# ChrisHird/ZLIB

Hardware: AMD Instinct MI355X
Metric: GiB/s raw input compressed (deflate level 6) (higher is better)
Workload: dtype u8

## Files before the change

### zlib_amd/csrc/zgpu_lz_parse.h

```cpp
#pragma once
#include "zgpu_common.h"

namespace zgpu {

#ifndef ZGPU_P2WIN
#define ZGPU_P2WIN 8192
#endif
constexpr uint32_t kP2Win = ZGPU_P2WIN, kP2Blk = kP2Win / 64;
constexpr uint32_t kP2Words = kChunkMax / 32, kP2Batch = 8, kP2Pair = 4, kP2Over = 8;
constexpr uint32_t kNone = 0xffffffffu;

struct ParseCtx {
    const uint2 *rec;
    uint32_t n, base, good, lazy, strategy;
    int slide_at;
    __device__ bool slid(uint32_t p) const { return (int)p >= slide_at; }
    __device__ uint32_t take(uint32_t p, uint32_t prev_len, uint2 r, uint32_t &dist) const
    {
        const uint32_t pick = (prev_len >= good && strategy != kRle) ? r.y : r.x;
        const uint32_t d = (pick >> 9) & 32767u;
        const bool nil = ((r.y >> 24) & 1u) && slid(p);
        const uint32_t len = nil ? 0u : (pick & 511u);
        const bool weak = len <= 5 && (strategy == kFiltered || (len == kMinMatch && d > kTooFar));
        const bool ok = prev_len < lazy && len > prev_len && !weak;
// ... 7 lines not shown
        uint32_t q = r + 1;
        for (;;) {
            uint32_t D2 = 0;
            const uint32_t L2 = take(q, L, rn, D2);
            if (L2 <= L) break;
            L = L2; D = D2; q++;
            rn = rec[q];
        }
        m = q - 1; len = L; dist = D;
    }
};

__device__ inline uint32_t wave_rol1(uint32_t v) { return (uint32_t)__builtin_amdgcn_update_dpp(0, (int)v, 0x134, 0xf, 0xf, false); }

__device__ inline uint32_t next_bit(const uint32_t *bits, uint32_t x, uint32_t nwords)
{
    uint32_t w = x >> 5;
    if (w >= nwords) return kNone;
    uint32_t v = bits[w] & (~0u << (x & 31u));
    while (v == 0) { if (++w >= nwords) return kNone; v = bits[w]; }
    return (w << 5) + (uint32_t)__builtin_ctz(v);
}

#if defined(ZGPU_P2_TIME) && !defined(ZGPU_PARSE_HEADER_ONLY)
__device__ unsigned long long p2_time[8];
extern "C" __attribute__((visibility("default"))) void zgpu_debug_p2_time(unsigned long long *out, int reset)
{
    unsigned long long z[8] = {};
    hipMemcpyFromSymbol(out, HIP_SYMBOL(p2_time), sizeof z);
    if (reset) hipMemcpyToSymbol(HIP_SYMBOL(p2_time), z, sizeof z);
}
#define P2_T(i) do { if (tid == 0) { const unsigned long long t_ = wall_clock64(); t_acc[i] += t_ - t_prev; t_prev = t_; } } while (0)
#define P2_T0() unsigned long long t_prev = wall_clock64(), t_acc[8] = {0, 0, 0, 0, 0, 0, 0, 0}
#define P2_TEND() do { if (tid == 0) for (int i_ = 0; i_ < 8; i_++) atomicAdd(&p2_time[i_], t_acc[i_]); } while (0)
#else
#define P2_T(i) do { } while (0)
#define P2_T0() do { } while (0)
#define P2_TEND() do { } while (0)
#endif

template <bool FUSED> __device__ inline uint32_t p2_ld(const uint32_t *p) { return FUSED ? __hip_atomic_load(p, __ATOMIC_RELAXED, __HIP_MEMORY_SCOPE_AGENT) : *p; }
constexpr uint32_t kP2OffJ = 0, kP2OffHAS = kP2Win * 2, kP2OffMARK = kP2OffHAS + kP2Words * 4, kP2OffCOV = kP2OffMARK + kP2Words * 4, kP2OffMAT = kP2OffCOV + kP2Words * 4,
                   kP2OffWbase = kP2OffMAT + kP2Words * 4, kP2OffVIS = kP2OffWbase + (kP2Words + 4) * 4, kP2OffEXITS = kP2OffVIS + kP2Win / 32 * 4, kP2OffWtot = kP2OffEXITS + 256,
                   kP2OffEntry = kP2OffWtot + 64, kP2LdsBytes = kP2OffEntry + 16;
constexpr uint32_t kP2Wins = kChunkMax / kP2Win, kP2OffEND = kP2LdsBytes, kP2LogLdsBytes = kP2OffEND + kP2Win * 2;
static_assert(kChunkMax % kP2Win == 0 && kP2Win - 1 + 255 + 258 <= 0xffffu, "whole windows; a game's end fits END");

}
```

### zlib_amd/csrc/zgpu_lz_parse_body.inc

```
{
    constexpr uint32_t kP2Own = kP2Win / kP2Threads;
    static_assert(kP2Own % kP2Batch == 0 && kP2Threads >= kP2Win / 32 && kP2Threads / 64 <= 16, "workgroup size");
    const uint32_t tid = threadIdx.x, lane = tid & 63, wave = tid >> 6;
    uint64_t lo; uint32_t n;
    chunk_span(g, c, lo, n);
    ParseCtx cx;
    cx.rec = LITE ? nullptr : recs + (size_t)c * kChunkMax;
    const uint32_t *gmv = LITE ? gmv_all + (size_t)c * kChunkMax : nullptr, *gsv = LITE ? gsv_all + (size_t)c * kP2Words : nullptr;
    cx.n = n; cx.base = chunk_base(g, c); cx.good = cfg.good; cx.lazy = cfg.lazy; cx.strategy = cfg.strategy;
    {
        const int room = (int)(2 * kWSize - cx.base), b0 = (int)n < room ? (int)n : room;
        const int a = b0 - (int)kMinLookahead + 1, b = (int)(kWSize + kMaxDist) - (int)cx.base;
        cx.slide_at = a > b ? a : b;
    }
    uint32_t *tok = tokens + (size_t)c * kChunkMax;
    const uint8_t *src = g.in + lo;
    const uint32_t nwords = (n + 31) >> 5;
    uint32_t t_h1 = n, t_e = 0;
    if (TILE) {
        uint64_t wb_; uint32_t nl_, h0_, ne_;
        tile_span(g, tg, c, wb_, nl_, h0_, t_h1, ne_);
        t_e = h0_ + tg.entry[g.chunk0 + c];
    }

    static_assert(!LOG || (LITE && !TILE), "the logs are what a chunk's walkers leave");
    P2_T0();
    for (uint32_t i = tid; i < kP2Words; i += kP2Threads) { MARK[i] = 0; COV[i] = 0; MAT[i] = 0; if (LOG) HAS[i] = 0; else if (LITE) HAS[i] = p2_ld<FUSED>(gsv + i); }
    const uint32_t *lpos2 = reinterpret_cast<const uint32_t *>(lpos);
    if (LOG) {
        constexpr uint32_t kRounds = kP2Win / 2 / kP2Threads;
        __syncthreads();
        for (uint32_t w = 0; w < kP2Wins; w++) {
            const uint32_t cw = (uint32_t)__builtin_amdgcn_readfirstlane((int)lcnt[w]);
            uint32_t pv[kRounds];
#pragma unroll
            for (uint32_t r = 0; r < kRounds; r++) { pv[r] = 0; if (r * kP2Threads * 2 < cw) pv[r] = p2_ld<FUSED>(lpos2 + w * (kP2Win / 2) + r * kP2Threads + tid); }
#pragma unroll
            for (uint32_t r = 0; r < kRounds; r++) {
                const uint32_t e = (r * kP2Threads + tid) * 2, p0 = pv[r] & 0xffffu, p1 = pv[r] >> 16;
                if (e < cw) atomicOr(&HAS[p0 >> 5], 1u << (p0 & 31u));
                if (e + 1 < cw) atomicOr(&HAS[p1 >> 5], 1u << (p1 & 31u));
            }
        }
    }
    if (!LITE) for (uint32_t p0 = 0; p0 < kChunkMax; p0 += kP2Threads * kP2Batch) {
        uint2 rv[kP2Batch];
#pragma unroll
        for (uint32_t u = 0; u < kP2Batch; u++) { const uint32_t p = p0 + u * kP2Threads + tid; rv[u] = p < n ? cx.rec[p] : make_uint2(0, 0); }
#pragma unroll
        for (uint32_t u = 0; u < kP2Batch; u++) {
            const uint32_t pw = p0 + u * kP2Threads, p = pw + tid;
            uint32_t d;
            const bool h = p < n && cx.take(p, kMinMatch - 1, rv[u], d) >= kMinMatch;
            const unsigned long long b = __builtin_amdgcn_ballot_w64(h);
            if (lane == 0) { HAS[(pw >> 5) + 2 * wave] = (uint32_t)b; HAS[(pw >> 5) + 2 * wave + 1] = (uint32_t)(b >> 32); }
        }
    }
    __syncthreads();
    if (tid == 0) {
        uint32_t x0 = (!TILE || t_e < t_h1) ? next_bit(HAS, t_e, nwords) : kNone;
        if (TILE && x0 != kNone && x0 >= t_h1) x0 = kNone;
        sh_entry = x0;
        if (TILE) sh_exit = t_e;
    }
    __syncthreads();
    P2_T(0);

    const uint32_t *TOK = COV;
    auto index_of = [&](uint32_t p) { return wbase[p >> 5] + (uint32_t)__builtin_popcount(TOK[p >> 5] & ~(~0u << (p & 31u))); };
    uint32_t tokbase = 0;
    uint32_t def_m = kNone, def_tok = 0;

    const uint32_t w_first = TILE ? t_e / kP2Win * kP2Win : 0u, w_lim = TILE ? (t_h1 + kTileSlack < n ? t_h1 + kTileSlack : n) : n;
    for (uint32_t w0 = w_first; w0 < w_lim; w0 += kP2Win) {
        const uint32_t wend = w0 + kP2Win;
        const uint32_t entry = sh_entry;
        uint32_t gm[kP2Own];
        uint32_t gp[kP2Own];
        uint32_t onp = 0;
#pragma unroll
        for (uint32_t i = 0; i < kP2Own; i++) { gm[i] = 0; gp[i] = 0; }
        auto pos_of = [&](uint32_t i) { return LOG ? gp[i] : w0 + i * kP2Threads + tid; };
        if (entry != kNone && entry < wend) {
            if (LOG) {
                const uint32_t cw = (uint32_t)__builtin_amdgcn_readfirstlane((int)lcnt[w0 / kP2Win]);
                const uint32_t *lp2 = lpos2 + w0 / 2, *lr = lrec + w0;
                uint32_t gv[kP2Own], gq[kP2Own];
#pragma unroll
                for (uint32_t i = 0; i < kP2Own; i++) {
                    gv[i] = 0; gq[i] = 0;
                    if (i * kP2Threads < cw) { const uint32_t e = i * kP2Threads + tid; gq[i] = p2_ld<FUSED>(lp2 + (e >> 1)); gv[i] = p2_ld<FUSED>(lr + e); }
                }
#pragma unroll
                for (uint32_t i = 0; i < kP2Own; i++) {
                    const bool v = i * kP2Threads + tid < cw;
                    const uint32_t p = (gq[i] >> ((tid & 1u) << 4)) & 0xffffu;
                    gm[i] = v ? gv[i] : 0u; gp[i] = v ? p : 0u;
                    if (v) {
                        const uint32_t end = p + (gv[i] >> 24) + ((gv[i] >> 15) & 511u), t = next_bit(HAS, end, nwords);
                        J[p - w0] = (uint16_t)(t < wend ? t - w0 : 0xffffu);
                        END[p - w0] = (uint16_t)(end - w0);
                    }
                }
            } else if (LITE) {
                uint32_t gv[kP2Own];
#pragma unroll
                for (uint32_t i = 0; i < kP2Own; i++) {
                    const uint32_t p = w0 + i * kP2Threads + tid;
#if defined(ZGPU_P2_EXP) && ZGPU_P2_EXP == 1
                    gv[i] = 0x00018001u;
#else
                    gv[i] = p < n ? p2_ld<FUSED>(gmv + p) : 0;
#endif
                }
#pragma unroll
                for (uint32_t i = 0; i < kP2Own; i++) {
                    const uint32_t p = w0 + i * kP2Threads + tid;
                    if (!(p < n && ((HAS[p >> 5] >> (p & 31u)) & 1u))) gv[i] = 0;
                }
#pragma unroll
                for (uint32_t i = 0; i < kP2Own; i++) {
                    const uint32_t xw = i * kP2Threads + tid, p = w0 + xw;
// ... 28 lines not shown
                        const uint32_t tx = wave_rol1(qx), ty = wave_rol1(qy);
                        ox = wave_rol1(ox); oy = wave_rol1(oy);
                        qx = lane == 63 ? ox : tx; qy = lane == 63 ? oy : ty;
                        uint2 rn;
                        rn.x = qx; rn.y = qy;
                        const bool far = live && sl >= 64 + kP2Over;
                        if (__builtin_amdgcn_ballot_w64(far)) { if (far) rn = cx.rec[p + j]; }
                        uint32_t D2 = D;
                        const uint32_t L2 = cx.take(p + j, L, rn, D2);
                        live = live && L2 > L;
                        L = live ? L2 : L; D = live ? D2 : D; j += live ? 1u : 0u;
                    }
                    uint32_t succ = 0xffffu;
                    if (hs) {
                        const uint32_t m = p + j - 1;
                        gm[ib + u] = ((m - p) << 24) | (L << 15) | D;
                        const uint32_t t = next_bit(HAS, m + L, nwords);
                        if (t < wend) succ = t - w0;
                    }
                    J[x] = (uint16_t)succ;
                }
            }
            }
            __syncthreads();
            P2_T(1);
            if (wave == 0) {
                const uint32_t bs = w0 + lane * kP2Blk, be = bs + kP2Blk;
                uint32_t v8[kP2Blk / 32];
#pragma unroll
                for (uint32_t j = 0; j < kP2Blk / 32; j++) v8[j] = 0;
                uint32_t x = next_bit(HAS, bs, nwords);
                if (x != kNone && x >= wend) x = kNone;
                while (x != kNone && x < be) {
                    const uint32_t wi = (x - bs) >> 5, bit = 1u << (x & 31u);
#pragma unroll
                    for (uint32_t j = 0; j < kP2Blk / 32; j++) v8[j] |= wi == j ? bit : 0u;
                    const uint32_t a2 = J[x - w0];
                    x = a2 == 0xffffu ? kNone : w0 + a2;
                }
#pragma unroll
                for (uint32_t j = 0; j < kP2Blk / 32; j++) VIS[lane * (kP2Blk / 32) + j] = v8[j];
                EXITS[lane] = x;
                __builtin_amdgcn_fence(__ATOMIC_SEQ_CST, "wavefront");
                __builtin_amdgcn_wave_barrier();
                uint32_t last = entry;
                bool ok;
// ... 108 lines not shown
            uint32_t tw = 0;
            if (tid < kP2Win / 32 && wd < nwords) {
                tw = ~COV[wd];
                if (wd == nwords - 1 && (n & 31u)) tw &= ~0u >> (32u - (n & 31u));
                if (TILE) {
                    const uint32_t xl = wend > t_h1 ? (sh_exit > t_h1 ? sh_exit : t_h1) : wend, p0 = wd << 5;
                    tw &= p0 + 32 <= t_e ? 0u : p0 >= t_e ? ~0u : ~0u << (t_e & 31u);
                    tw &= p0 >= xl ? 0u : p0 + 32 <= xl ? ~0u : ~0u >> (32u - (xl & 31u));
                }
            }
            const uint32_t cnt = (uint32_t)__builtin_popcount(tw);
            uint32_t x = cnt;
#pragma unroll
            for (int d = 1; d < 64; d <<= 1) { const uint32_t y = __shfl_up(x, d); if ((int)lane >= d) x += y; }
            if (lane == 63) wave_tot[wave] = x;
            __syncthreads();
            uint32_t b = tokbase + x - cnt, tot = 0;
            for (uint32_t w = 0; w < kP2Win / 32 / 64; w++) { const uint32_t t = wave_tot[w]; tot += t; if (w < wave) b += t; }
            if (tid < kP2Win / 32) { wbase[wd] = b; COV[wd] = tw; }
            tokbase += tot;
            __syncthreads();
        }
        P2_T(4);
        if (def_m != kNone) { tok[index_of(def_m)] = def_tok; def_m = kNone; }
#pragma unroll
        for (uint32_t ib = 0; ib < kP2Own; ib += kP2Batch) {
            uint32_t lit[kP2Batch];
            bool li[kP2Batch];
#pragma unroll
            for (uint32_t u = 0; u < kP2Batch; u++) {
                const uint32_t p = w0 + (ib + u) * kP2Threads + tid, bit = 1u << (p & 31u);
                li[u] = p < n && (TOK[p >> 5] & bit) && !(MAT[p >> 5] & bit);
                lit[u] = 0;
                if (p < n) lit[u] = src[p];
            }
#pragma unroll
            for (uint32_t u = 0; u < kP2Batch; u++) {
                const uint32_t p = w0 + (ib + u) * kP2Threads + tid;
                if (li[u]) tok[index_of(p)] = tok_lit(lit[u]);
                const uint32_t gv = (!LOG && ((onp >> (ib + u)) & 1u)) ? gm[ib + u] : 0u;
                if (gv) {
                    const uint32_t m = p + (gv >> 24), t = tok_match(gv & 32767u, ((gv >> 15) & 511u) - kMinMatch);
                    if (m < wend) tok[index_of(m)] = t; else { def_m = m; def_tok = t; }
                }
            }
        }
        if (LOG) {
#pragma unroll
            for (uint32_t i = 0; i < kP2Own; i++) {
                const uint32_t gv = ((onp >> i) & 1u) ? gm[i] : 0u;
                if (gv) {
                    const uint32_t m = gp[i] + (gv >> 24), t = tok_match(gv & 32767u, ((gv >> 15) & 511u) - kMinMatch);
                    if (m < wend) tok[index_of(m)] = t; else { def_m = m; def_tok = t; }
                }
            }
        }
        P2_T(5);
    }
    const uint32_t ntok = tokbase, nw_done = ((n + kP2Win - 1) / kP2Win) * (kP2Win / 32);
    __syncthreads();

    if (TILE) { if (tid == 0) { meta[c].ntok = ntok; meta[c].in_bytes = (sh_exit > t_h1 ? sh_exit : t_h1) - t_e; } }
    else if (tid == 0) {
        uint32_t nostore = 0, nblk = 0, block_start = 0;
        for (uint32_t b = 0;; b++) {
            const uint32_t e = (b + 1) * kBlockTokens - 1;
            if (e >= ntok) break;
            uint32_t lo_w = 0, hi_w = nw_done;
            while (hi_w - lo_w > 1) { const uint32_t mid = (lo_w + hi_w) >> 1; if (wbase[mid] <= e) lo_w = mid; else hi_w = mid; }
            uint32_t v = TOK[lo_w];
            for (uint32_t s2 = e - wbase[lo_w]; s2; s2--) v &= v - 1;
            const uint32_t pe = (lo_w << 5) + (uint32_t)__builtin_ctz(v);
            const bool is_mat = (MAT[pe >> 5] >> (pe & 31u)) & 1u;
            if (!is_mat && pe == n - 1) { nostore |= kFullFinalBlock; break; }
            uint32_t ns = pe + 1;
            if (is_mat) { ns = next_bit(TOK, pe + 1, nwords); if (ns == kNone) ns = n; }
            if (cx.slid(pe + 1) && block_start + cx.base < kWSize) nostore |= 1u << nblk;
            nblk++; block_start = ns;
// ... 8 lines not shown
```

### zlib_amd/csrc/zgpu_lz_sorted.hip

```cpp
#include "zgpu_common.h"
#include "zgpu_engine.h"
#include "zgpu_deflate_batch_plan.h"
#define ZGPU_PARSE_HEADER_ONLY
#include "zgpu_lz_parse.h"
#include <cstdlib>
#include "../../include/zamd_gpu.h"

#include <atomic>
static std::atomic<int> g_inject_sort_fault{0};
extern "C" __attribute__((visibility("default"))) void zgpu_debug_inject_sort_fault(void) { g_inject_sort_fault.store(1); }

namespace zgpu {

__device__ inline uint32_t lds_off(const void *p) { return (uint32_t)(uintptr_t)(const __attribute__((address_space(3))) void *)p; }
__device__ inline void lds_st32(uint32_t a, uint32_t v) { asm volatile("ds_write_b32 %0, %1" ::"v"(a), "v"(v) : "memory"); }
__device__ inline void lds_st16(uint32_t a, uint32_t v) { asm volatile("ds_write_b16 %0, %1" ::"v"(a), "v"(v) : "memory"); }
__device__ inline void lds_max32(uint32_t a, uint32_t v) { asm volatile("ds_max_u32 %0, %1" ::"v"(a), "v"(v) : "memory"); }
__device__ inline uint32_t lds_ld32(uint32_t a) { uint32_t v; asm volatile("ds_read_b32 %0, %1\n\ts_waitcnt lgkmcnt(0)" : "=v"(v) : "v"(a) : "memory"); return v; }
__device__ inline uint32_t lds_ld16(uint32_t a) { uint32_t v; asm volatile("ds_read_u16 %0, %1\n\ts_waitcnt lgkmcnt(0)" : "=v"(v) : "v"(a) : "memory"); return v; }

__device__ inline void lds_st8(uint32_t a, uint32_t v) { asm volatile("ds_write_b8 %0, %1" ::"v"(a), "v"(v) : "memory"); }
__device__ inline uint32_t lds_ld8(uint32_t a) { uint32_t v; asm volatile("ds_read_u8 %0, %1\n\ts_waitcnt lgkmcnt(0)" : "=v"(v) : "v"(a) : "memory"); return v; }

constexpr uint32_t kSuperS = 1024;
// ... 639 lines not shown
            uint32_t full = 0, snap = 0, flags = 0;
            if (key_seen) {
                const uint32_t kb = 4095u - ((key_seen >> 31) ? (key_seen >> 16) & 0xfffu : key_seen & 0xfffu);
                full = best | ((p - (uint32_t)sp[-1 - (int)kb]) << 9);
            }
            if (snapkey) {
                const uint32_t ks = 4095u - ((snapkey >> 31) ? (snapkey >> 16) & 0xfffu : snapkey & 0xfffu);
                const uint32_t sl = (snapkey >> 31) ? snapkey & 0x1ffu : snapkey >> 16;
                snap = sl | ((p - (uint32_t)sp[-1 - (int)ks]) << 9);
            }
            if (p + base == kWSize + kMaxDist && avail != 0 && (uint32_t)sp[-1] + base == kWSize) flags = 1;
            rec[p] = make_uint2(full | ((uint32_t)d8[p] << 24), snap | (flags << 24));
        }
        blk = blk_nx;
    }
}

#ifndef ZGPU_WTRIG
#define ZGPU_WTRIG 48
#endif
#ifndef ZGPU_WBLK
#define ZGPU_WBLK 64
#endif
#ifndef ZGPU_WNEU_SHIFT
#define ZGPU_WNEU_SHIFT 0
#endif
#ifndef ZGPU_WFOLD_AT
#define ZGPU_WFOLD_AT 64
#endif
constexpr uint32_t kWFoldAt = ZGPU_WFOLD_AT;
constexpr uint32_t kWThreads = 512, kWWaves = kWThreads / 64, kWBlk = ZGPU_WBLK, kWTrig = ZGPU_WTRIG, kWNeuShift = ZGPU_WNEU_SHIFT;
constexpr uint32_t kWNeuBytes = (kChunkMax >> kWNeuShift) / 8;
constexpr uint32_t kWOffLcnt = kM3DataLds + 16 + kWNeuBytes + kWWaves * kM3WaveLds;
constexpr uint32_t kWLds = kWOffLcnt + kP2Wins * 4;
static_assert(2 * kWLds <= 160 * 1024, "two walker workgroups per CU");
enum : uint32_t { W_NEED = 0, W_LIMBO = 1, W_READY = 2, W_SEARCH = 3, W_DONE = 4 };
#ifdef ZGPU_WALK_STATS
__device__ unsigned long long walk_stats[8];
extern "C" __attribute__((visibility("default"))) void zgpu_debug_walk_stats(unsigned long long *out, int reset)
{
    unsigned long long z[8] = {};
    hipMemcpyFromSymbol(out, HIP_SYMBOL(walk_stats), sizeof z);
    if (reset) hipMemcpyToSymbol(HIP_SYMBOL(walk_stats), z, sizeof z);
}
#define W_STAT(i, v) do { const unsigned long long v_ = (unsigned long long)(v); if (lane == 0) atomicAdd(&walk_stats[i], v_); } while (0)
__device__ unsigned long long walk_log_stats[2];
extern "C" __attribute__((visibility("default"))) void zgpu_debug_walk_log_stats(unsigned long long *out, int reset)
{
    unsigned long long z[2] = {};
    hipMemcpyFromSymbol(out, HIP_SYMBOL(walk_log_stats), sizeof z);
    if (reset) hipMemcpyToSymbol(HIP_SYMBOL(walk_log_stats), z, sizeof z);
}
#else
#define W_STAT(i, v) do { } while (0)
#endif
#ifdef ZGPU_WALK_TIME
__device__ unsigned long long walk_time[8];
extern "C" __attribute__((visibility("default"))) void zgpu_debug_walk_time(unsigned long long *out, int reset)
{
    unsigned long long z[8] = {};
    hipMemcpyFromSymbol(out, HIP_SYMBOL(walk_time), sizeof z);
    if (reset) hipMemcpyToSymbol(HIP_SYMBOL(walk_time), z, sizeof z);
}
#define W_T0() unsigned long long wt_prev = __builtin_readcyclecounter(), wt_fold = 0, wt_lds = 0, wt_take = 0, wt_acc[8] = {0, 0, 0, 0, 0, 0, 0, 0}
#define W_T(i) do { const unsigned long long t_ = __builtin_readcyclecounter(); wt_acc[i] += t_ - wt_prev - ((i) == 1 ? wt_fold + wt_lds + wt_take : 0); \
                    if ((i) == 1) { wt_acc[2] += wt_fold; wt_acc[3] += wt_lds; wt_acc[7] += wt_take; } wt_fold = wt_lds = wt_take = 0; wt_prev = t_; } while (0)
#define W_TF(stmt) do { const unsigned long long f0_ = __builtin_readcyclecounter(); stmt; wt_fold += __builtin_readcyclecounter() - f0_; } while (0)
#define W_TL(stmt) do { const unsigned long long f0_ = __builtin_readcyclecounter(); stmt; wt_lds += __builtin_readcyclecounter() - f0_; } while (0)
#define W_TK(stmt) do { const unsigned long long f0_ = __builtin_readcyclecounter(); asm volatile("s_waitcnt vmcnt(0)" ::: "memory"); stmt; wt_take += __builtin_readcyclecounter() - f0_; } while (0)
#define W_TEND() do { if (lane == 0) for (int i_ = 0; i_ < 8; i_++) atomicAdd(&walk_time[i_], wt_acc[i_]); } while (0)
#else
#define W_T0() do { } while (0)
#define W_T(i) do { } while (0)
#define W_TF(stmt) stmt
#define W_TL(stmt) stmt
#define W_TK(stmt) stmt
#define W_TEND() do { } while (0)
#endif
__device__ inline uint32_t add_w1(uint32_t b, uint32_t w) { uint32_t r; asm("v_add_u32_sdwa %0, %1, %2 dst_sel:DWORD dst_unused:UNUSED_PAD src0_sel:DWORD src1_sel:WORD_1" : "=v"(r) : "v"(b), "v"(w)); return r; }
__device__ inline uint32_t add_w0(uint32_t b, uint32_t w) { uint32_t r; asm("v_add_u32_sdwa %0, %1, %2 dst_sel:DWORD dst_unused:UNUSED_PAD src0_sel:DWORD src1_sel:WORD_0" : "=v"(r) : "v"(b), "v"(w)); return r; }
__device__ inline uint32_t or_w1(uint32_t b, uint32_t w) { uint32_t r; asm("v_or_b32_sdwa %0, %1, %2 dst_sel:DWORD dst_unused:UNUSED_PAD src0_sel:DWORD src1_sel:WORD_1" : "=v"(r) : "v"(b), "v"(w)); return r; }
__device__ inline uint32_t and_or(uint32_t w, uint32_t m, uint32_t b) { uint32_t r; asm("v_and_or_b32 %0, %1, %2, %3" : "=v"(r) : "v"(w), "s"(m), "v"(b)); return r; }
__device__ inline uint32_t sel_mask(unsigned long long m, uint32_t if_set, uint32_t if_clear) { uint32_t r; asm("v_cndmask_b32_e64 %0, %1, %2, %3" : "=v"(r) : "v"(if_clear), "v"(if_set), "s"(m)); return r; }

template <uint32_t T>
__device__ inline void tile_exits(uint8_t *pl, const uint32_t *gm, const uint32_t *gs, uint32_t h0, uint32_t h1, uint32_t nent, uint16_t *exits, uint32_t tid)
{
    constexpr uint32_t kWords = kChunkMax / 32;
    static_assert(kWords % T == 0 && T % 64 == 0 && T <= 1024, "workgroup size");
    uint32_t *HAS = reinterpret_cast<uint32_t *>(pl);
    uint16_t *wcnt = reinterpret_cast<uint16_t *>(pl + kWords * 4);
    uint32_t *wtot = reinterpret_cast<uint32_t *>(pl + kWords * 6);
    uint16_t *N = reinterpret_cast<uint16_t *>(pl + kWords * 6 + 64);
    constexpr uint32_t kCapNodes = (kM3DataLds - (kWords * 6 + 64)) / 2;
    static_assert(kCapNodes < 0x8000u && kCapNodes > kTileH1 / 3, "a path's game starts are three positions apart at least; different paths' need not be");
    const uint32_t lane = tid & 63, wave = tid >> 6;
    constexpr uint32_t per = kWords / T;
    uint32_t sum = 0, cnt[per];
#pragma unroll
    for (uint32_t i = 0; i < per; i++) {
// ... 78 lines not shown
    uint32_t *ctrl = lds + kM3DataLds / 4;
    uint32_t *NEU = ctrl + 4;
    uint32_t *lcnt = lds + kWOffLcnt / 4;
    const uint32_t c = blockIdx.x, tid = threadIdx.x, lane = tid & 63, wave = tid >> 6;
    const uint32_t ring = (uint32_t)__builtin_amdgcn_readfirstlane(lds_off(lds) + kM3DataLds + 16 + kWNeuBytes + wave * kM3WaveLds), slot = ring + kRing * 4;
    uint64_t lo; uint32_t n;
    chunk_span(g, c, lo, n);
    const uint8_t *src = g.in + lo;
    const uint16_t *S = S_all + (size_t)c * kSStride + kSPad;
    const uint32_t *ir = ir_all + (size_t)c * kChunkMax;
    uint32_t *gm = gm_all + (size_t)c * kChunkMax, *gs = gs_all + (size_t)c * (kChunkMax / 32);
    uint32_t *lrec = gm; uint16_t *lpos = reinterpret_cast<uint16_t *>(gs_all) + (size_t)c * kChunkMax;
    uint32_t th0 = 0, th1 = n, tnent = 0, tnent_all = 0, nil_local = ~0u;
    uint32_t base = chunk_base(g, c);
    if (TILE) {
        uint64_t wb; uint32_t nl;
        tile_span(g, tg, c, wb, nl, th0, th1, tnent);
        tnent_all = tnent;
        if (tnent > th1 - th0) tnent = th1 - th0;
        base = (tg.abs0_nil && tg.abs0 + wb == 0) ? 0u : 1u;
        if (tg.nil_pos >= wb && tg.nil_pos - wb < kChunkMax) nil_local = (uint32_t)(tg.nil_pos - wb);
    }
    const uint32_t npos = n >= 3 ? n - 2 : 0;
    stage_chunk<kWThreads>(src, n, d32, tid);
    for (uint32_t i = tid; i < kChunkMax / 32; i += kWThreads) { if (i < kWNeuBytes / 4) NEU[i] = 0; if (!FUSE) gs[i] = 0; }
    if (tid < 8) d32[(kChunkMax + 64) / 4 + tid] = 0xffffffffu;
    if (tid == 0) ctrl[0] = 0;
    if (FUSE && tid < kP2Wins) lcnt[tid] = 0;
    __syncthreads();
    int slide_at;
    {
        const int room = (int)(2 * kWSize - base), b0 = (int)n < room ? (int)n : room;
        const int a = b0 - (int)kMinLookahead + 1, b = (int)(kWSize + kMaxDist) - (int)base;
        slide_at = a > b ? a : b;
    }
    const uint32_t chainF = cfg.chain, chainQ = cfg.chain >> 2, dbase = lds_off(d32), nblk = TILE ? tnent + (th1 - th0 - tnent + kWBlk - 1) / kWBlk : (n + kWBlk - 1) / kWBlk;
    const uint32_t wlim = TILE ? th1 : n;
    const bool vexact = (chainF & 7u) != 0 || (chainQ & 7u) != 0 || cfg.strategy == kRle;
    uint32_t lanebits = lane << 16;
    const uint32_t dummy = ring + (kRing - 1) * 4;
    uint32_t st = W_NEED, x = 0, handL = kMinMatch - 1, handM = 0, handD = 0, gstart = 0;
    uint32_t irx = 0, irn = 0, irE = 0, irl = 0;
    bool haveE = false;
    uint32_t rem = 0, best = kMinMatch - 1, key_seen = 0, sentinel = 0, boff = dbase + 1;
    uint32_t sw0 = 0, sw1 = 0;
    int gi = -(int)kSPad;
    uint32_t firstb = 0;
    uint4 G0 = make_uint4(0, 0, 0, 0), G1 = G0, G2 = G0, G3 = G0, F0 = G0, F1 = G0, F2 = G0, F3 = G0;
    uint32_t left = 0;
    bool cont = false;
    unsigned long long amask = 0, jmask = 0;
    uint32_t tail = 0;

    auto fold = [&]() {
        const uint32_t cnt = tail < 64 ? tail : 64;
        W_STAT(5, 1); W_STAT(6, cnt);
        tail = (uint32_t)__builtin_amdgcn_readfirstlane(tail - cnt);
        const uint32_t e = lds_ld32(ring + ((tail + lane) << 2));
        const uint32_t q = e & 0xffffu, o = (e >> 16) & 63u, qa = dbase + q;
// ... 9 lines not shown
        if (lane < cnt) {
            const uint32_t look = n - po, cap = look < kMaxMatch ? look : kMaxMatch, nice = cfg.nice < look ? cfg.nice : look;
            const bool reach = po - q <= kMaxDist - ((e >> 22) & 1u ? 0u : 1u) && q + base >= 1u;
            uint32_t l = 0;
            while ((xa | xb) == 0 && l + 8 < cap) {
                l += 8;
                lds_cmp8(qa + l, dbase + po + l, xa, xb);
            }
            uint32_t len = xa ? l + ((uint32_t)__builtin_ctz(xa) >> 3) : xb ? l + 4 + ((uint32_t)__builtin_ctz(xb) >> 3) : l + 8;
            len = len < cap ? len : cap;
            if (len >= kMinMatch && reach) lds_max32(slot + o * 4, (len >= nice && len > (e >> 23)) ? (0x80000000u | (q << 9) | len) : ((len << 16) | q));
        }
        const uint32_t key = lds_ld32(slot + lane * 4);
        if (key != key_seen) {
            key_seen = key;
            best = (key >> 31) ? key & 0x1ffu : key >> 16;
            boff = dbase + best - 1;
        }
        amask &= ~mask_lt_i32((int)key, 0);
    };
    auto gload = [&](int gi) -> uint4 { gi = gi < -(int)kSPad ? -(int)kSPad : gi; return reinterpret_cast<const U128u *>(S + gi)->v; };

    W_T0();
    W_T(3);
    for (;;) {
        while (tail) fold();
        W_T(4);
        if (cont && (key_seen >> 31)) cont = false;
        const bool fin = st == W_SEARCH && !(((amask | jmask) >> lane) & 1ull) && !cont;
        W_STAT(2, 1); W_STAT(3, __popcll(__builtin_amdgcn_ballot_w64(fin || st == W_LIMBO || st == W_NEED)));
        if (st == W_LIMBO) { irx = irl; st = W_READY; }
        uint32_t y = 0, irY = 0, rec = 0;
        bool toN = false, haveIr = false, emit = false;
        if (fin) {
            uint32_t len = kMinMatch - 1, dist = 0;
            if (key_seen != sentinel) {
                const bool nz = key_seen >> 31;
                len = nz ? key_seen & 0x1ffu : key_seen >> 16;
                dist = x - (nz ? (key_seen >> 9) & 0xffffu : key_seen & 0xffffu);
            }
            if (len <= 5 && (cfg.strategy == kFiltered || (len == kMinMatch && dist > kTooFar))) len = kMinMatch - 1;
            if (len > handL) {
                if (handL < kMinMatch) gstart = x;
                handL = len; handD = dist; handM = x;
                if (len < cfg.lazy && x + 1 < npos) { x = x + 1; irx = irn; st = W_READY; }
                else emit = true;
                haveE = false;
            } else if (handL >= kMinMatch) emit = true;
            else { y = x + 1; irY = irn; toN = haveIr = true; }
            if (emit) {
                rec = ((handM - gstart) << 24) | (handL << 15) | handD;
                if (!FUSE) {
                    gm[gstart] = rec;
// ... 22 lines not shown
            const uint32_t at = lw * kP2Win + lslot;
            lrec[at] = rec; lpos[at] = (uint16_t)gstart;
        }
        if (toN) {
            st = W_NEED;
            if (y < wlim && (!meet || !(yold & ybit))) {
                x = y;
                if (haveIr) { irx = irY; st = W_READY; }
                else { irl = y < npos ? ir[y] : 0; st = W_LIMBO; W_STAT(7, 1); }
            }
        }
        W_T(5);
        {
            const unsigned long long nm = __builtin_amdgcn_ballot_w64(st == W_NEED);
            if (nm) {
                const int first = __builtin_ctzll(nm);
                uint32_t b0 = 0;
                if ((int)lane == first) b0 = atomicAdd(&ctrl[0], (uint32_t)__popcll(nm));
                b0 = (uint32_t)__builtin_amdgcn_readlane((int)b0, first);
                if (st == W_NEED) {
                    const uint32_t b = b0 + __builtin_amdgcn_mbcnt_hi((uint32_t)(nm >> 32), __builtin_amdgcn_mbcnt_lo((uint32_t)nm, 0));
                    if (b >= nblk) st = W_DONE;
                    else {
                        const uint32_t y2 = TILE ? (b < tnent ? th0 + b : th0 + tnent + (b - tnent) * kWBlk) : b * kWBlk, bit = 1u << ((y2 >> kWNeuShift) & 31u);
                        if (!(atomicOr(&NEU[(y2 >> kWNeuShift) >> 5], bit) & bit)) { x = y2; handL = kMinMatch - 1; irl = y2 < npos ? ir[y2] : 0; st = W_LIMBO; }
                    }
                }
            }
        }
        W_T(6);
        bool fresh = false;
        if (st == W_READY) {
            const uint32_t seed = handL, idx = irx & 0xffffu, rank = irx >> 16, budget = seed >= cfg.good ? (chainQ ? chainQ : 0xffffu) : chainF;
            uint32_t avail = (x < npos && seed < cfg.lazy) ? (rank < budget ? rank : budget) : 0;
            irn = x + 1 < npos ? ir[x + 1] : 0;
            if (seed >= kMinMatch) { const uint32_t E = handM + handL; irE = E < npos ? ir[E] : 0; haveE = true; }
            if (TILE) {
                if (x == nil_local && avail != 0 && x - (uint32_t)S[idx - 1] == kMaxDist) avail = 0;
                if (cfg.strategy == kHuffmanOnly) avail = 0;
                if (cfg.strategy == kRle && avail != 0) avail = x - (uint32_t)S[idx - 1] == 1 ? 1u : 0u;
            }
            else if (x + base == kWSize + kMaxDist && avail != 0 && (int)x >= slide_at && (uint32_t)S[idx - 1] + base == kWSize) avail = 0;
            best = seed; sentinel = (seed << 16) | 0xffffu; key_seen = sentinel; boff = dbase + best - 1;
            lds_st32(slot + lane * 4, sentinel);
            sw0 = tw0; sw1 = tw1;
            lanebits = (lane << 16) | (seed << 23);
            rem = avail; firstb = 1u << 22;
            gi = (int)idx - 8;
            st = W_SEARCH;
            fresh = avail != 0;
            W_STAT(4, 1);
        }
        if (cont) { cont = false; fresh = true; }
        jmask = __builtin_amdgcn_ballot_w64(fresh);
        if (fresh) {
            F0 = gload(gi);
            if (rem > 8) F1 = gload(gi - 8);
            if (rem > 16) F2 = gload(gi - 16);
            if (rem > 24) F3 = gload(gi - 24);
            gi -= 32;
        }
        W_T(0);
        if (__builtin_amdgcn_ballot_w64(st != W_DONE) == 0) { W_TEND(); break; }
        const unsigned long long smask = __builtin_amdgcn_ballot_w64(st == W_SEARCH);
        const uint32_t idle = (uint32_t)__popcll(__builtin_amdgcn_ballot_w64(st == W_LIMBO || st == W_NEED));

        for (bool first = true;; first = false) {
            const unsigned long long amask0 = amask;
            if (amask) {
                W_STAT(0, 1);
                uint32_t bb[8], a[8], boff_e, as;
                boff_e = boff; as = boff + x;
                if (!vexact) {
                    const uint32_t boff_i = dbase + kChunkMax + 8u;
                    G0.x = sel_mask(amask0, G0.x, 0u); G0.y = sel_mask(amask0, G0.y, 0u); G0.z = sel_mask(amask0, G0.z, 0u); G0.w = sel_mask(amask0, G0.w, 0u);
                    boff_e = sel_mask(amask0, boff, boff_i); as = sel_mask(amask0, as, boff_i + 64u);
                }
                a[0] = add_w1(boff_e, G0.w); a[1] = add_w0(boff_e, G0.w); a[2] = add_w1(boff_e, G0.z); a[3] = add_w0(boff_e, G0.z);
                a[4] = add_w1(boff_e, G0.y); a[5] = add_w0(boff_e, G0.y); a[6] = add_w1(boff_e, G0.x); a[7] = add_w0(boff_e, G0.x);
                uint32_t hi[8], s0, s1;
                W_TL(
                    asm volatile("ds_read_u8 %0, %18\n\tds_read_u8 %8, %18 offset:1\n\tds_read_u8 %1, %19\n\tds_read_u8 %9, %19 offset:1\n\t"
                                 "ds_read_u8 %2, %20\n\tds_read_u8 %10, %20 offset:1\n\tds_read_u8 %3, %21\n\tds_read_u8 %11, %21 offset:1\n\t"
                                 "ds_read_u8 %4, %22\n\tds_read_u8 %12, %22 offset:1\n\tds_read_u8 %5, %23\n\tds_read_u8 %13, %23 offset:1\n\t"
                                 "ds_read_u8 %6, %24\n\tds_read_u8 %14, %24 offset:1\n\tds_read_u8 %7, %25\n\tds_read_u8 %15, %25 offset:1\n\t"
                                 "ds_read_u8 %16, %26\n\tds_read_u8 %17, %26 offset:1\n\t"
// ... 54 lines not shown
                    while (tail >= kWFoldAt) W_TF(fold());
                }
                amask &= mask_gt_u32(rem, 8u);
                firstb = sel_mask(amask0, 0u, firstb);
            }
            G0 = G1; G1 = G2; G2 = G3;
            left = left ? left - 1 : 0;
            if (first && jmask) {
                W_TK(if ((jmask >> lane) & 1ull) { G0 = F0; G1 = F1; G2 = F2; G3 = F3; left = 4; });
            }
            rem = sel_mask(amask0, rem > 8 ? rem - 8 : 0, rem);
            {
                const unsigned long long cm = amask & mask_eq_u32(left, 0u);
                cont = cont || ((cm >> lane) & 1ull);
                amask &= ~cm;
            }
            amask |= jmask; jmask = 0;
            if (amask == 0 || (uint32_t)__popcll(smask & ~amask) + idle >= kWTrig) break;
        }
        W_T(1);
    }
    if (TILE) {
        __syncthreads();
        tile_exits<kWThreads>(reinterpret_cast<uint8_t *>(lds), gm, gs, th0, th1, tnent_all, tg.exits + (size_t)c * kTileExitStride, tid);
    }
    if (FUSE) {
        __syncthreads();
#ifdef ZGPU_WALK_STATS
        if (tid < kP2Wins) { atomicAdd(&walk_log_stats[0], (unsigned long long)lcnt[tid]); atomicMax(&walk_log_stats[1], (unsigned long long)lcnt[tid]); }
#endif
        constexpr uint32_t kP2Threads = kWThreads;
        constexpr bool LITE = true, FUSED = true, TILE = false, LOG = true;
        const uint2 *recs = nullptr;
        const uint32_t *gmv_all = nullptr, *gsv_all = nullptr;
        uint8_t *pl = reinterpret_cast<uint8_t *>(lds);
        uint16_t *const J = reinterpret_cast<uint16_t *>(pl + kP2OffJ);
        uint32_t *const HAS = reinterpret_cast<uint32_t *>(pl + kP2OffHAS), *const MARK = reinterpret_cast<uint32_t *>(pl + kP2OffMARK), *const COV = reinterpret_cast<uint32_t *>(pl + kP2OffCOV),
                 *const MAT = reinterpret_cast<uint32_t *>(pl + kP2OffMAT), *const wbase = reinterpret_cast<uint32_t *>(pl + kP2OffWbase), *const VIS = reinterpret_cast<uint32_t *>(pl + kP2OffVIS),
                 *const EXITS = reinterpret_cast<uint32_t *>(pl + kP2OffEXITS), *const wave_tot = reinterpret_cast<uint32_t *>(pl + kP2OffWtot);
        uint32_t &sh_entry = *reinterpret_cast<uint32_t *>(pl + kP2OffEntry), &sh_exit = *reinterpret_cast<uint32_t *>(pl + kP2OffEntry + 4);
        uint16_t *const END = reinterpret_cast<uint16_t *>(pl + kP2OffEND);
#include "zgpu_lz_parse_body.inc"
    }
}

struct __attribute__((packed, aligned(1))) U128b { uint4 v; };
enum : uint32_t { F_IR = 0, F_GROUP, F_CAND, F_EXT, F_DONE };

__device__ inline uint32_t first_diff16(uint4 a, uint4 b)
{
// ... 254 lines not shown
```

Baseline: 29.40.

## Prefetch next window's logs, batch token stores, and taper walker block sizes

The parse body now prefetches the next window's log entries and the current window's literal bytes while the current window is processed, so global loads overlap with compute. Token stores are batched, with indices computed first and then stored, and gp is packed two positions per register to cut VGPR use. The walker also splits the end of each chunk into smaller 32- and 16-byte blocks to shorten tail latency. Extra timing and stat instrumentation is added. These changes trade more live registers, from prefetched arrays and unrolled log loads, for less memory stall and less tail imbalance.

```diff
diff --git a/zlib_amd/csrc/zgpu_lz_parse.h b/zlib_amd/csrc/zgpu_lz_parse.h
--- a/zlib_amd/csrc/zgpu_lz_parse.h
+++ b/zlib_amd/csrc/zgpu_lz_parse.h
@@ -53,7 +53,9 @@
     return (w << 5) + (uint32_t)__builtin_ctz(v);
 }
 
-#if defined(ZGPU_P2_TIME) && !defined(ZGPU_PARSE_HEADER_ONLY)
+#ifdef ZGPU_P2_TIME
+#ifndef ZGPU_PARSE_HEADER_ONLY
+#define P2_TIME_ARR p2_time
 __device__ unsigned long long p2_time[8];
 extern "C" __attribute__((visibility("default"))) void zgpu_debug_p2_time(unsigned long long *out, int reset)
 {
@@ -61,9 +63,10 @@
     hipMemcpyFromSymbol(out, HIP_SYMBOL(p2_time), sizeof z);
     if (reset) hipMemcpyToSymbol(HIP_SYMBOL(p2_time), z, sizeof z);
 }
+#endif
 #define P2_T(i) do { if (tid == 0) { const unsigned long long t_ = wall_clock64(); t_acc[i] += t_ - t_prev; t_prev = t_; } } while (0)
 #define P2_T0() unsigned long long t_prev = wall_clock64(), t_acc[8] = {0, 0, 0, 0, 0, 0, 0, 0}
-#define P2_TEND() do { if (tid == 0) for (int i_ = 0; i_ < 8; i_++) atomicAdd(&p2_time[i_], t_acc[i_]); } while (0)
+#define P2_TEND() do { if (tid == 0) for (int i_ = 0; i_ < 7; i_++) atomicAdd(&P2_TIME_ARR[i_], t_acc[i_]); } while (0)
 #else
 #define P2_T(i) do { } while (0)
 #define P2_T0() do { } while (0)
diff --git a/zlib_amd/csrc/zgpu_lz_parse_body.inc b/zlib_amd/csrc/zgpu_lz_parse_body.inc
--- a/zlib_amd/csrc/zgpu_lz_parse_body.inc
+++ b/zlib_amd/csrc/zgpu_lz_parse_body.inc
@@ -27,19 +27,34 @@
     P2_T0();
     for (uint32_t i = tid; i < kP2Words; i += kP2Threads) { MARK[i] = 0; COV[i] = 0; MAT[i] = 0; if (LOG) HAS[i] = 0; else if (LITE) HAS[i] = p2_ld<FUSED>(gsv + i); }
     const uint32_t *lpos2 = reinterpret_cast<const uint32_t *>(lpos);
+    uint32_t nq[kP2Own], nv[kP2Own];
+    auto log_fetch = [&](uint32_t w0n, uint32_t tid) {
+        const uint32_t cw = (uint32_t)__builtin_amdgcn_readfirstlane((int)lcnt[w0n / kP2Win]);
+        const uint32_t *lp2 = lpos2 + w0n / 2, *lr = lrec + w0n;
+#pragma unroll
+        for (uint32_t i = 0; i < kP2Own; i++) {
+            nq[i] = 0; nv[i] = 0;
+            if (i * kP2Threads < cw) { const uint32_t e = i * kP2Threads + tid; nq[i] = p2_ld<FUSED>(lp2 + (e >> 1)); nv[i] = p2_ld<FUSED>(lr + e); }
+        }
+    };
     if (LOG) {
         constexpr uint32_t kRounds = kP2Win / 2 / kP2Threads;
         __syncthreads();
-        for (uint32_t w = 0; w < kP2Wins; w++) {
-            const uint32_t cw = (uint32_t)__builtin_amdgcn_readfirstlane((int)lcnt[w]);
-            uint32_t pv[kRounds];
-#pragma unroll
-            for (uint32_t r = 0; r < kRounds; r++) { pv[r] = 0; if (r * kP2Threads * 2 < cw) pv[r] = p2_ld<FUSED>(lpos2 + w * (kP2Win / 2) + r * kP2Threads + tid); }
+        log_fetch(0, tid);
+        uint32_t pv[kP2Wins][kRounds], cw[kP2Wins];
+#pragma unroll
+        for (uint32_t a = 0; a < kP2Wins; a++) {
+            cw[a] = (uint32_t)__builtin_amdgcn_readfirstlane((int)lcnt[a]);
+#pragma unroll
+            for (uint32_t r = 0; r < kRounds; r++) { pv[a][r] = 0; if (r * kP2Threads * 2 < cw[a]) pv[a][r] = p2_ld<FUSED>(lpos2 + a * (kP2Win / 2) + r * kP2Threads + tid); }
+        }
+#pragma unroll
+        for (uint32_t a = 0; a < kP2Wins; a++) {
 #pragma unroll
             for (uint32_t r = 0; r < kRounds; r++) {
-                const uint32_t e = (r * kP2Threads + tid) * 2, p0 = pv[r] & 0xffffu, p1 = pv[r] >> 16;
-                if (e < cw) atomicOr(&HAS[p0 >> 5], 1u << (p0 & 31u));
-                if (e + 1 < cw) atomicOr(&HAS[p1 >> 5], 1u << (p1 & 31u));
+                const uint32_t e = (r * kP2Threads + tid) * 2, p0 = pv[a][r] & 0xffffu, p1 = pv[a][r] >> 16;
+                if (e < cw[a]) atomicOr(&HAS[p0 >> 5], 1u << (p0 & 31u));
+                if (e + 1 < cw[a]) atomicOr(&HAS[p1 >> 5], 1u << (p1 & 31u));
             }
         }
     }
@@ -72,32 +87,36 @@
     uint32_t def_m = kNone, def_tok = 0;
 
     const uint32_t w_first = TILE ? t_e / kP2Win * kP2Win : 0u, w_lim = TILE ? (t_h1 + kTileSlack < n ? t_h1 + kTileSlack : n) : n;
+    const uint32_t tid_all = tid;
     for (uint32_t w0 = w_first; w0 < w_lim; w0 += kP2Win) {
         const uint32_t wend = w0 + kP2Win;
+        uint32_t tid = tid_all;
+        if (LOG) asm volatile("" : "+v"(tid));
         const uint32_t entry = sh_entry;
         uint32_t gm[kP2Own];
-        uint32_t gp[kP2Own];
+        uint32_t gp[kP2Own / 2];
         uint32_t onp = 0;
 #pragma unroll
-        for (uint32_t i = 0; i < kP2Own; i++) { gm[i] = 0; gp[i] = 0; }
-        auto pos_of = [&](uint32_t i) { return LOG ? gp[i] : w0 + i * kP2Threads + tid; };
-        if (entry != kNone && entry < wend) {
+        for (uint32_t i = 0; i < kP2Own; i++) { gm[i] = 0; gp[i >> 1] = 0; }
+        auto pos_of = [&](uint32_t i) { return LOG ? (gp[i >> 1] >> ((i & 1u) << 4)) & 0xffffu : w0 + i * kP2Threads + tid; };
+        uint32_t litw[kP2Own];
+        auto win_fetch = [&]() {
+#pragma unroll
+            for (uint32_t i = 0; i < kP2Own; i++) { const uint32_t p = w0 + i * kP2Threads + tid; litw[i] = 0; if (p < n) litw[i] = src[p]; }
+            if (wend < n) log_fetch(wend, tid);
+        };
+        const bool has_path = entry != kNone && entry < wend;
+        if (has_path) {
             if (LOG) {
                 const uint32_t cw = (uint32_t)__builtin_amdgcn_readfirstlane((int)lcnt[w0 / kP2Win]);
-                const uint32_t *lp2 = lpos2 + w0 / 2, *lr = lrec + w0;
-                uint32_t gv[kP2Own], gq[kP2Own];
-#pragma unroll
-                for (uint32_t i = 0; i < kP2Own; i++) {
-                    gv[i] = 0; gq[i] = 0;
-                    if (i * kP2Threads < cw) { const uint32_t e = i * kP2Threads + tid; gq[i] = p2_ld<FUSED>(lp2 + (e >> 1)); gv[i] = p2_ld<FUSED>(lr + e); }
-                }
 #pragma unroll
                 for (uint32_t i = 0; i < kP2Own; i++) {
                     const bool v = i * kP2Threads + tid < cw;
-                    const uint32_t p = (gq[i] >> ((tid & 1u) << 4)) & 0xffffu;
-                    gm[i] = v ? gv[i] : 0u; gp[i] = v ? p : 0u;
+                    const uint32_t p = (nq[i] >> ((tid & 1u) << 4)) & 0xffffu;
+                    const uint32_t gvi = nv[i];
+                    gm[i] = v ? gvi : 0u; gp[i >> 1] |= (v ? p : 0u) << ((i & 1u) << 4);
                     if (v) {
-                        const uint32_t end = p + (gv[i] >> 24) + ((gv[i] >> 15) & 511u), t = next_bit(HAS, end, nwords);
+                        const uint32_t end = p + (gvi >> 24) + ((gvi >> 15) & 511u), t = next_bit(HAS, end, nwords);
                         J[p - w0] = (uint16_t)(t < wend ? t - w0 : 0xffffu);
                         END[p - w0] = (uint16_t)(end - w0);
                     }
@@ -172,6 +191,9 @@
                 }
             }
             }
+        }
+        if (LOG) win_fetch();
+        if (has_path) {
             __syncthreads();
             P2_T(1);
             if (wave == 0) {
@@ -326,22 +348,30 @@
             __syncthreads();
         }
         P2_T(4);
+        auto tok_put = [&](uint32_t idx, uint32_t v) { *reinterpret_cast<uint32_t *>(reinterpret_cast<uint8_t *>(tok) + (idx << 2)) = v; };
         if (def_m != kNone) { tok[index_of(def_m)] = def_tok; def_m = kNone; }
 #pragma unroll
         for (uint32_t ib = 0; ib < kP2Own; ib += kP2Batch) {
-            uint32_t lit[kP2Batch];
+            uint32_t lit[kP2Batch], ix[kP2Batch];
             bool li[kP2Batch];
 #pragma unroll
             for (uint32_t u = 0; u < kP2Batch; u++) {
                 const uint32_t p = w0 + (ib + u) * kP2Threads + tid, bit = 1u << (p & 31u);
                 li[u] = p < n && (TOK[p >> 5] & bit) && !(MAT[p >> 5] & bit);
                 lit[u] = 0;
-                if (p < n) lit[u] = src[p];
+                if (LOG) lit[u] = litw[ib + u];
+                else if (p < n) lit[u] = src[p];
+                ix[u] = LOG ? index_of(p) : 0u;
+            }
+            if (LOG) {
+#pragma unroll
+                for (uint32_t u = 0; u < kP2Batch; u++) asm volatile("" : "+v"(lit[u]), "+v"(ix[u]));
             }
 #pragma unroll
             for (uint32_t u = 0; u < kP2Batch; u++) {
                 const uint32_t p = w0 + (ib + u) * kP2Threads + tid;
-                if (li[u]) tok[index_of(p)] = tok_lit(lit[u]);
+                if (LOG) { if (li[u]) tok_put(ix[u], tok_lit(lit[u])); }
+                else if (li[u]) tok[index_of(p)] = tok_lit(lit[u]);
                 const uint32_t gv = (!LOG && ((onp >> (ib + u)) & 1u)) ? gm[ib + u] : 0u;
                 if (gv) {
                     const uint32_t m = p + (gv >> 24), t = tok_match(gv & 32767u, ((gv >> 15) & 511u) - kMinMatch);
@@ -351,13 +381,20 @@
         }
         if (LOG) {
 #pragma unroll
-            for (uint32_t i = 0; i < kP2Own; i++) {
-                const uint32_t gv = ((onp >> i) & 1u) ? gm[i] : 0u;
-                if (gv) {
-                    const uint32_t m = gp[i] + (gv >> 24), t = tok_match(gv & 32767u, ((gv >> 15) & 511u) - kMinMatch);
-                    if (m < wend) tok[index_of(m)] = t; else { def_m = m; def_tok = t; }
-                }
-            }
+                for (uint32_t ib = 0; ib < kP2Own; ib += kP2Batch) {
+                    uint32_t mx[kP2Batch], mt[kP2Batch];
+#pragma unroll
+                    for (uint32_t u = 0; u < kP2Batch; u++) {
+                        const uint32_t gv = ((onp >> (ib + u)) & 1u) ? gm[ib + u] : 0u, m = pos_of(ib + u) + (gv >> 24);
+                        mt[u] = gv ? tok_match(gv & 32767u, ((gv >> 15) & 511u) - kMinMatch) : 0u;
+                        mx[u] = kNone;
+                        if (gv) { if (m < wend) mx[u] = index_of(m); else { def_m = m; def_tok = mt[u]; } }
+                    }
+#pragma unroll
+                    for (uint32_t u = 0; u < kP2Batch; u++) asm volatile("" : "+v"(mx[u]), "+v"(mt[u]));
+#pragma unroll
+                    for (uint32_t u = 0; u < kP2Batch; u++) if (mx[u] != kNone) tok_put(mx[u], mt[u]);
+                }
         }
         P2_T(5);
     }
diff --git a/zlib_amd/csrc/zgpu_lz_sorted.hip b/zlib_amd/csrc/zgpu_lz_sorted.hip
--- a/zlib_amd/csrc/zgpu_lz_sorted.hip
+++ b/zlib_amd/csrc/zgpu_lz_sorted.hip
@@ -685,6 +685,12 @@
 #ifndef ZGPU_WBLK
 #define ZGPU_WBLK 64
 #endif
+#ifndef ZGPU_WTAPER32
+#define ZGPU_WTAPER32 16384
+#endif
+#ifndef ZGPU_WTAPER16
+#define ZGPU_WTAPER16 4096
+#endif
 #ifndef ZGPU_WNEU_SHIFT
 #define ZGPU_WNEU_SHIFT 0
 #endif
@@ -694,19 +700,43 @@
 constexpr uint32_t kWFoldAt = ZGPU_WFOLD_AT;
 constexpr uint32_t kWThreads = 512, kWWaves = kWThreads / 64, kWBlk = ZGPU_WBLK, kWTrig = ZGPU_WTRIG, kWNeuShift = ZGPU_WNEU_SHIFT;
 constexpr uint32_t kWNeuBytes = (kChunkMax >> kWNeuShift) / 8;
+constexpr uint32_t kWTaper32 = ZGPU_WTAPER32, kWTaper16 = ZGPU_WTAPER16, kWTaperMin = kWThreads * kWBlk;
+static_assert(kWTaper16 <= kWTaper32 && kWTaper32 <= kWTaperMin && kWTaper32 % 64 == 0 && kWTaper16 % 64 == 0, "the tapered end lies inside a chunk that has one");
+static_assert((kWTaper32 == 0 && kWTaper16 == 0) || kWBlk == 64, "blocks of 32 and 16 follow blocks of 64");
+static_assert(kWTaper32 == 0 || kWNeuShift <= (kWTaper16 ? 4 : 5), "a short block's start must be a meeting position of its own, or the walker in front passes through it and the block is never taken");
+struct WalkTaper {
+    uint32_t b32, b16, n64, n32, nblk;
+    __host__ __device__ explicit WalkTaper(uint32_t n)
+    {
+        const bool on = n > kWTaperMin && kWTaper32 != 0;
+        b32 = on ? (n - kWTaper32) & ~63u : n;
+        b16 = on ? (n - kWTaper16) & ~31u : n;
+        n64 = on ? b32 / 64 : (n + kWBlk - 1) / kWBlk; n32 = (b16 - b32) / 32;
+        nblk = n64 + n32 + (n - b16 + 15) / 16;
+    }
+    __host__ __device__ uint32_t start(uint32_t b) const { return b < n64 ? b * kWBlk : b < n64 + n32 ? b32 + (b - n64) * 32 : b16 + (b - n64 - n32) * 16; }
+};
+extern "C" __attribute__((visibility("default"))) void zgpu_walk_block_map(uint32_t n, uint32_t *out)
+{
+    const WalkTaper t(n);
+    out[0] = t.b32; out[1] = t.b16; out[2] = t.nblk;
+}
 constexpr uint32_t kWOffLcnt = kM3DataLds + 16 + kWNeuBytes + kWWaves * kM3WaveLds;
 constexpr uint32_t kWLds = kWOffLcnt + kP2Wins * 4;
 static_assert(2 * kWLds <= 160 * 1024, "two walker workgroups per CU");
 enum : uint32_t { W_NEED = 0, W_LIMBO = 1, W_READY = 2, W_SEARCH = 3, W_DONE = 4 };
 #ifdef ZGPU_WALK_STATS
-__device__ unsigned long long walk_stats[8];
+__device__ unsigned long long walk_stats[12];
 extern "C" __attribute__((visibility("default"))) void zgpu_debug_walk_stats(unsigned long long *out, int reset)
 {
-    unsigned long long z[8] = {};
+    unsigned long long z[12] = {};
     hipMemcpyFromSymbol(out, HIP_SYMBOL(walk_stats), sizeof z);
     if (reset) hipMemcpyToSymbol(HIP_SYMBOL(walk_stats), z, sizeof z);
 }
 #define W_STAT(i, v) do { const unsigned long long v_ = (unsigned long long)(v); if (lane == 0) atomicAdd(&walk_stats[i], v_); } while (0)
+#define W_SOUT0() bool ws_out = false
+#define W_SLIVE() do { W_STAT(ws_out ? 9 : 8, __popcll(__builtin_amdgcn_ballot_w64(st != W_DONE))); W_STAT(ws_out ? 11 : 10, 1); } while (0)
+#define W_SOUT() do { ws_out = ws_out || __builtin_amdgcn_ballot_w64(st == W_DONE) != 0; } while (0)
 __device__ unsigned long long walk_log_stats[2];
 extern "C" __attribute__((visibility("default"))) void zgpu_debug_walk_log_stats(unsigned long long *out, int reset)
 {
@@ -716,29 +746,46 @@
 }
 #else
 #define W_STAT(i, v) do { } while (0)
+#define W_SOUT0() do { } while (0)
+#define W_SLIVE() do { } while (0)
+#define W_SOUT() do { } while (0)
 #endif
 #ifdef ZGPU_WALK_TIME
-__device__ unsigned long long walk_time[8];
+__device__ unsigned long long walk_time[10];
 extern "C" __attribute__((visibility("default"))) void zgpu_debug_walk_time(unsigned long long *out, int reset)
 {
-    unsigned long long z[8] = {};
+    unsigned long long z[10] = {};
     hipMemcpyFromSymbol(out, HIP_SYMBOL(walk_time), sizeof z);
     if (reset) hipMemcpyToSymbol(HIP_SYMBOL(walk_time), z, sizeof z);
 }
-#define W_T0() unsigned long long wt_prev = __builtin_readcyclecounter(), wt_fold = 0, wt_lds = 0, wt_take = 0, wt_acc[8] = {0, 0, 0, 0, 0, 0, 0, 0}
+#define W_T0() unsigned long long wt_prev = __builtin_readcyclecounter(), wt_fold = 0, wt_lds = 0, wt_take = 0, wt_out = 0, wt_acc[10] = {0, 0, 0, 0, 0, 0, 0, 0, 0, 0}
 #define W_T(i) do { const unsigned long long t_ = __builtin_readcyclecounter(); wt_acc[i] += t_ - wt_prev - ((i) == 1 ? wt_fold + wt_lds + wt_take : 0); \
                     if ((i) == 1) { wt_acc[2] += wt_fold; wt_acc[3] += wt_lds; wt_acc[7] += wt_take; } wt_fold = wt_lds = wt_take = 0; wt_prev = t_; } while (0)
 #define W_TF(stmt) do { const unsigned long long f0_ = __builtin_readcyclecounter(); stmt; wt_fold += __builtin_readcyclecounter() - f0_; } while (0)
 #define W_TL(stmt) do { const unsigned long long f0_ = __builtin_readcyclecounter(); stmt; wt_lds += __builtin_readcyclecounter() - f0_; } while (0)
 #define W_TK(stmt) do { const unsigned long long f0_ = __builtin_readcyclecounter(); asm volatile("s_waitcnt vmcnt(0)" ::: "memory"); stmt; wt_take += __builtin_readcyclecounter() - f0_; } while (0)
-#define W_TEND() do { if (lane == 0) for (int i_ = 0; i_ < 8; i_++) atomicAdd(&walk_time[i_], wt_acc[i_]); } while (0)
+#define W_TOUT() do { if (!wt_out && __builtin_amdgcn_ballot_w64(st == W_DONE)) wt_out = wt_prev; } while (0)
+#define W_TEXIT() do { wt_acc[8] = wt_prev - wt_out; } while (0)
+#define W_TEND() do { wt_acc[9] = __builtin_readcyclecounter() - wt_prev; if (lane == 0) for (int i_ = 0; i_ < 10; i_++) atomicAdd(&walk_time[i_], wt_acc[i_]); } while (0)
 #else
 #define W_T0() do { } while (0)
 #define W_T(i) do { } while (0)
 #define W_TF(stmt) stmt
 #define W_TL(stmt) stmt
 #define W_TK(stmt) stmt
+#define W_TOUT() do { } while (0)
+#define W_TEXIT() do { } while (0)
 #define W_TEND() do { } while (0)
+#endif
+#ifdef ZGPU_P2_TIME
+__device__ unsigned long long p2_fused_time[8];
+extern "C" __attribute__((visibility("default"))) void zgpu_debug_p2_fused_time(unsigned long long *out, int reset)
+{
+    unsigned long long z[8] = {};
+    hipMemcpyFromSymbol(out, HIP_SYMBOL(p2_fused_time), sizeof z);
+    if (reset) hipMemcpyToSymbol(HIP_SYMBOL(p2_fused_time), z, sizeof z);
+}
+#define P2_TIME_ARR p2_fused_time
 #endif
 __device__ inline uint32_t add_w1(uint32_t b, uint32_t w) { uint32_t r; asm("v_add_u32_sdwa %0, %1, %2 dst_sel:DWORD dst_unused:UNUSED_PAD src0_sel:DWORD src1_sel:WORD_1" : "=v"(r) : "v"(b), "v"(w)); return r; }
 __device__ inline uint32_t add_w0(uint32_t b, uint32_t w) { uint32_t r; asm("v_add_u32_sdwa %0, %1, %2 dst_sel:DWORD dst_unused:UNUSED_PAD src0_sel:DWORD src1_sel:WORD_0" : "=v"(r) : "v"(b), "v"(w)); return r; }
@@ -863,6 +910,9 @@
         if (tg.nil_pos >= wb && tg.nil_pos - wb < kChunkMax) nil_local = (uint32_t)(tg.nil_pos - wb);
     }
     const uint32_t npos = n >= 3 ? n - 2 : 0;
+#ifdef ZGPU_P2_TIME
+    const unsigned long long p2_t_in = wall_clock64();
+#endif
     stage_chunk<kWThreads>(src, n, d32, tid);
     for (uint32_t i = tid; i < kChunkMax / 32; i += kWThreads) { if (i < kWNeuBytes / 4) NEU[i] = 0; if (!FUSE) gs[i] = 0; }
     if (tid < 8) d32[(kChunkMax + 64) / 4 + tid] = 0xffffffffu;
@@ -875,7 +925,8 @@
         const int a = b0 - (int)kMinLookahead + 1, b = (int)(kWSize + kMaxDist) - (int)base;
         slide_at = a > b ? a : b;
     }
-    const uint32_t chainF = cfg.chain, chainQ = cfg.chain >> 2, dbase = lds_off(d32), nblk = TILE ? tnent + (th1 - th0 - tnent + kWBlk - 1) / kWBlk : (n + kWBlk - 1) / kWBlk;
+    const WalkTaper taper(n);
+    const uint32_t chainF = cfg.chain, chainQ = cfg.chain >> 2, dbase = lds_off(d32), nblk = TILE ? tnent + (th1 - th0 - tnent + kWBlk - 1) / kWBlk : taper.nblk;
     const uint32_t wlim = TILE ? th1 : n;
     const bool vexact = (chainF & 7u) != 0 || (chainQ & 7u) != 0 || cfg.strategy == kRle;
     uint32_t lanebits = lane << 16;
@@ -931,6 +982,7 @@
     auto gload = [&](int gi) -> uint4 { gi = gi < -(int)kSPad ? -(int)kSPad : gi; return reinterpret_cast<const U128u *>(S + gi)->v; };
 
     W_T0();
+    W_SOUT0();
     W_T(3);
     for (;;) {
         while (tail) fold();
@@ -938,6 +990,7 @@
         if (cont && (key_seen >> 31)) cont = false;
         const bool fin = st == W_SEARCH && !(((amask | jmask) >> lane) & 1ull) && !cont;
         W_STAT(2, 1); W_STAT(3, __popcll(__builtin_amdgcn_ballot_w64(fin || st == W_LIMBO || st == W_NEED)));
+        W_SLIVE();
         if (st == W_LIMBO) { irx = irl; st = W_READY; }
         uint32_t y = 0, irY = 0, rec = 0;
         bool toN = false, haveIr = false, emit = false;
@@ -1006,13 +1059,14 @@
                     const uint32_t b = b0 + __builtin_amdgcn_mbcnt_hi((uint32_t)(nm >> 32), __builtin_amdgcn_mbcnt_lo((uint32_t)nm, 0));
                     if (b >= nblk) st = W_DONE;
                     else {
-                        const uint32_t y2 = TILE ? (b < tnent ? th0 + b : th0 + tnent + (b - tnent) * kWBlk) : b * kWBlk, bit = 1u << ((y2 >> kWNeuShift) & 31u);
+                        const uint32_t y2 = TILE ? (b < tnent ? th0 + b : th0 + tnent + (b - tnent) * kWBlk) : taper.start(b), bit = 1u << ((y2 >> kWNeuShift) & 31u);
                         if (!(atomicOr(&NEU[(y2 >> kWNeuShift) >> 5], bit) & bit)) { x = y2; handL = kMinMatch - 1; irl = y2 < npos ? ir[y2] : 0; st = W_LIMBO; }
                     }
                 }
             }
         }
         W_T(6);
+        W_TOUT(); W_SOUT();
         bool fresh = false;
         if (st == W_READY) {
             const uint32_t seed = handL, idx = irx & 0xffffu, rank = irx >> 16, budget = seed >= cfg.good ? (chainQ ? chainQ : 0xffffu) : chainF;
@@ -1045,7 +1099,7 @@
             gi -= 32;
         }
         W_T(0);
-        if (__builtin_amdgcn_ballot_w64(st != W_DONE) == 0) { W_TEND(); break; }
+        if (__builtin_amdgcn_ballot_w64(st != W_DONE) == 0) { W_TEXIT(); break; }
         const unsigned long long smask = __builtin_amdgcn_ballot_w64(st == W_SEARCH);
         const uint32_t idle = (uint32_t)__popcll(__builtin_amdgcn_ballot_w64(st == W_LIMBO || st == W_NEED));
 
@@ -1146,10 +1200,15 @@
     }
     if (TILE) {
         __syncthreads();
+        W_TEND();
         tile_exits<kWThreads>(reinterpret_cast<uint8_t *>(lds), gm, gs, th0, th1, tnent_all, tg.exits + (size_t)c * kTileExitStride, tid);
     }
     if (FUSE) {
         __syncthreads();
+        W_TEND();
+#ifdef ZGPU_P2_TIME
+        if (tid == 0) atomicAdd(&p2_fused_time[7], wall_clock64() - p2_t_in);
+#endif
 #ifdef ZGPU_WALK_STATS
         if (tid < kP2Wins) { atomicAdd(&walk_log_stats[0], (unsigned long long)lcnt[tid]); atomicMax(&walk_log_stats[1], (unsigned long long)lcnt[tid]); }
 #endif
```

Result: faster. 30.90 (median of 6 runs) (+5.1%).
